# AndrewCullacino/handwritten-chinese-ocr-samples

Hardware: AMD Instinct MI355X
Metric: text-lines/sec (1x128x2000 synth) greedy decode (higher is better)
Workload: dtype f16 (f32 accumulate); 1 GPU; BASELINE configs[1]: 64 x 1x128x2000 uint8 lines, random-init hctr checkpoint (C=7358), forward + greedy CTC decode, labels to host; global_lines=64, lines_per_gpu=64, width=2000, classes=7358, checkpoint=random, parallelism=batch-shard x1

## Files before the change

### handwritten-chinese-ocr-samples_amd/csrc/engine.cpp

```cpp
#include "../../include/hctr_hip.h"
#include "kernels.h"

#include <algorithm>
#include <cfloat>
#include <cmath>
#include <cstdarg>
#include <cstdio>
#include <cstring>
#include <map>
#include <new>
#include <string>
#include <vector>

using namespace hctr;

namespace {

constexpr int kImgH = 128;
constexpr int kFeat = 2048;
constexpr double kBnEps = 1e-5;
constexpr int kStagePlanes[4] = {128, 256, 512, 512};
constexpr int kStageBlocks[4] = {2, 4, 5, 1};
constexpr int kStageH[5] = {128, 64, 32, 16, 8};
constexpr int64_t kDefaultMaxCols = 131072;

std::string g_create_error;

struct HostTensor {
    std::vector<float> data;
    std::vector<int64_t> shape;
    mutable bool used = false;
};

struct ConvW {
    half_t* w = nullptr;
    float* bias = nullptr;
    int cin = 0, cout = 0, coutPad = 0, taps = 0;
};

struct SeW {
    float* w1 = nullptr;
    float* w2 = nullptr;
    int c = 0;
};

struct BlockW {
    ConvW conv1, conv2, ds;
    SeW se;
    bool has_ds = false;
};

struct Workspace {
    int B = 0, W = 0, Wa = 0;
    void* img = nullptr;
    int32_t* widths = nullptr;
    half_t* s0 = nullptr;
    half_t* x[5] = {};
    half_t* p[5][3] = {};
    half_t* headin = nullptr;
    float* logits = nullptr;
    float* se_part = nullptr;
    float* se_scale = nullptr;
    float* se_border = nullptr;
    float* se_mean = nullptr;
    int32_t* se_counter = nullptr;
    int32_t* colidx = nullptr;
    float* amax_val = nullptr;
    int32_t* amax_idx = nullptr;
    int32_t* labels = nullptr;
    int32_t* lengths = nullptr;
    float* psum = nullptr;
    float* blank_logit = nullptr;
    float* row_thr = nullptr;
    int32_t* emit_cnt = nullptr;
    int32_t* emit_list = nullptr;
    double* esum = nullptr;
    int32_t* overflow = nullptr;
    int32_t* bm_idx = nullptr;
    float* bm_lp = nullptr;
    float* bm_bl = nullptr;
    float* bm_st = nullptr;
    int32_t* bm_cnt = nullptr;
    int32_t* tile_ctrs = nullptr;
    float* amax_val2 = nullptr;
    float* amax_abs = nullptr;
    float* col_margin = nullptr;
    float* col_abs = nullptr;
    float* line_guard = nullptr;
    int features = 0;
    bool split = false;
    bool aliased = false;
};

enum WsFeature { WS_S0 = 1, WS_LOGITS = 2, WS_BEAM = 4, WS_GUARD = 8 };

struct WeightSet {
    float* stem_w = nullptr;
    float* stem_b = nullptr;
// ... 311 lines not shown
    half_t* pool4[4] = {};
    auto layout = [&](bool alias) {
        ws = Workspace();
        ws.B = B; ws.W = W; ws.features = feat; ws.split = c->split; ws.Wa = Wa; ws.aliased = alias;
        off = 0;
        slots.clear();
        auto A = [&](auto** out, size_t count) {
            slots.emplace_back((void**)out, off);
            off += (std::max<size_t>(count * sizeof(**out), 16) + 255) & ~(size_t)255;
        };
        A((char**)&ws.img, cols * kImgH * 4);
        A(&ws.widths, (size_t)B);
        int cin = 64;
        size_t se_max = 0, pool_elems = 0;
        for (int s = 1; s <= 4; ++s) {
            const int H = kStageH[s], planes = kStagePlanes[s - 1];
            if (!alias) {
                A(&ws.x[s], (size_t)act_elems(B, H, Wa, cin * m));
                const int nbuf = (s == 4) ? 2 : 3;
                for (int i = 0; i < nbuf; ++i) A(&ws.p[s][i], (size_t)act_elems(B, H, Wa, planes * m));
            }
            pool_elems = std::max(pool_elems, (size_t)act_elems(B, H, Wa, std::max(cin, planes) * m));
            se_max = std::max(se_max, (size_t)B * (H / 8) * tilesW * planes);
            cin = planes;
        }
        if (alias)
            for (int i = 0; i < 4; ++i) A(&pool4[i], pool_elems);
        A(&ws.headin, cols * kFeat * m);
        A(&ws.se_part, se_max);
        A(&ws.se_scale, (size_t)B * 512);
        A(&ws.se_border, (size_t)B * 5 * 8 * 512);
        A(&ws.se_mean, (size_t)B * 512);
        A(&ws.se_counter, (size_t)B);
        A(&ws.colidx, cols);
        const size_t P = (size_t)head_parts_max(c);
        A(&ws.amax_val, cols * P);
        A(&ws.amax_idx, cols * P);
        A(&ws.labels, cols);
        A(&ws.lengths, (size_t)B);
        A(&ws.tile_ctrs, (size_t)64 * 8);
        if (feat & WS_S0) A(&ws.s0, (size_t)act_elems(B, 128, Wa, 64 * m));
        if (feat & WS_LOGITS) A(&ws.logits, cols * c->cpad);
        if (feat & WS_GUARD) {
            A(&ws.amax_val2, cols * P);
            A(&ws.amax_abs, cols * P);
            A(&ws.col_margin, cols);
            A(&ws.col_abs, cols);
            A(&ws.line_guard, (size_t)2 * B);
        }
        if (feat & WS_BEAM) {
            A(&ws.psum, P * cols);
            A(&ws.blank_logit, cols);
            A(&ws.row_thr, 2 * cols);
            A(&ws.emit_cnt, cols);
            A(&ws.esum, P * cols);
            A(&ws.overflow, (size_t)1);
            A(&ws.bm_idx, cols * kBeamMaxK);
            A(&ws.bm_lp, cols * kBeamMaxK);
            A(&ws.bm_bl, cols);
            A(&ws.bm_st, 2 * cols);
            A(&ws.bm_cnt, cols);
            A(&ws.emit_list, cols * kBeamCap * 2);
        }
    };
    bool alias = c->ws_alias == 1;
    layout(alias);
// ... 15 lines not shown
        c->arena = nullptr; c->arena_cap = 0;
        c->ws = Workspace();
        const size_t want = off + off / 16;
        void* p = nullptr;
        hipError_t e = hipMalloc(&p, want);
        if (e != hipSuccess) e = hipMalloc(&p, off);
        if (e != hipSuccess)
            return fail(c, HCTR_ERR_NOMEM, "hipMalloc(%zu bytes) for the workspace of %d lines x %d columns failed: %s", off,
                        B, W, hipGetErrorString(e));
        c->arena = (char*)p;
        c->arena_cap = e == hipSuccess && want >= off ? want : off;
        ++c->arena_reallocs;
        fresh = true;
    }
    for (auto& sl : slots) *sl.first = c->arena + sl.second;
    if (ws.aliased) {
        for (int s = 1; s <= 4; ++s) {
            ws.x[s] = pool4[0];
            for (int i = 0; i < ((s == 4) ? 2 : 3); ++i) ws.p[s][i] = pool4[1 + i];
        }
    }
    if (c->ws.aliased != ws.aliased) same_shape = false;
    auto zero_act = [&](half_t* p, int H, int C) { return launch_zero_borders(p, B, H, W, Wa, C * m, c->stream); };
    if (fresh || !same_shape) {
        int ci = 64;
        for (int s = 1; s <= 4 && !ws.aliased; ++s) {
            const int H = kStageH[s], planes = kStagePlanes[s - 1];
            HIP_TRY(c, zero_act(ws.x[s], H, ci));
            const int nbuf = (s == 4) ? 2 : 3;
            for (int i = 0; i < nbuf; ++i) HIP_TRY(c, zero_act(ws.p[s][i], H, planes));
            ci = planes;
        }
        HIP_TRY(c, hipMemsetAsync(ws.se_counter, 0, (size_t)B * 4, c->stream));
        ++c->ws_recarves;
    }
    if (ws.s0 && (fresh || !same_shape || !c->ws.s0)) HIP_TRY(c, zero_act(ws.s0, 128, 64));
    c->ws = ws;
    return HCTR_OK;
}

struct Prof {
    hctr_ctx* c;
    bool on;
    explicit Prof(hctr_ctx* ctx) : c(ctx), on(ctx->profiling) {}
    hipEvent_t ev() {
        if (c->ev_used == c->ev_pool.size()) {
            hipEvent_t e;
            (void)hipEventCreate(&e);
            c->ev_pool.push_back(e);
        }
        return c->ev_pool[c->ev_used++];
    }
    void begin(const char* name) {
        if (!on) return;
        ProfEntry pe{name, ev(), ev()};
        (void)hipEventRecord(pe.e0, c->stream);
        c->prof.push_back(pe);
    }
    void end() {
        if (!on) return;
        (void)hipEventRecord(c->prof.back().e1, c->stream);
    }
};

inline void prof_reset(hctr_ctx* c) {
    if (c->profiling) { c->prof.clear(); c->ev_used = 0; }
// ... 50 lines not shown
    if (ds) {
        if (tile != TILE_HALO4 || !se_scale || resid || ds->cin % kBK != 0 || ds->coutPad != cw.coutPad)
            return fail(c, HCTR_ERR_STATE, "conv %s: downsample fusion not applicable", name);
        a.ds_x = ds_in; a.ds_w = ds->w; a.ds_bias = ds->bias; a.ds_cin = ds->cin;
        a.ds_in_sh = ws.Wa * ds->cin;
        a.ds_in_sb = (int64_t)(in.H + 2) * ws.Wa * ds->cin;
    }
    a.mtiles = ws.B * a.tilesH * a.tilesW;
    a.ntiles = cw.coutPad / conv_tile_couts(tile);
    if (c->persist_dynamic && c->conv_seq < 64) a.tile_counter = ws.tile_ctrs + 8 * c->conv_seq++;
    if (c->stamp_buf && c->stamp_layer == name && (tile == TILE_HALO4 || tile == TILE_HALO4_8x32) &&
        (int64_t)a.mtiles * a.ntiles <= c->stamp_cap) {
        a.stamps = c->stamp_buf;
        c->stamp_n = (int64_t)a.mtiles * a.ntiles;
    }
    static const char* dbg_layer = getenv("HCTR_DBG_LAYER");
    if (dbg_layer && strcmp(dbg_layer, name) == 0)
        if (const char* e = getenv("HCTR_DBG")) a.dbg = atoi(e);
    pf.begin(name);
    if (stem_img_f32 >= 0) {
        if (tile != TILE_64x256 || cw.taps != 9 || cw.cin != 64 || cw.coutPad != 64 || c->split)
            return fail(c, HCTR_ERR_STATE, "conv %s: stem fusion not applicable", name);
        a.img = ws.img; a.img_f32 = stem_img_f32; a.img_widths = stem_widths ? ws.widths : nullptr;
        a.stem_w = c->wts().stem_w; a.stem_b = c->wts().stem_b;
        HIP_TRY(c, launch_stem_conv0_2(a, c->stream));
    } else {
        HIP_TRY(c, launch_conv(a, tile, cw.taps, false, c->stream));
    }
    pf.end();
    return HCTR_OK;
}

int run_block(hctr_ctx* c, Prof& pf, const std::string& name, const BlockW& bw, ActDesc in, half_t* t,
              half_t* o, half_t* r, int planes) {
    const Workspace& ws = c->ws;
    const int H = in.H;
    auto tiles_of = [&](const ConvW& cw) {
        const ConvTile t = pick_tile(c, cw, H);
        return (H / conv_tile_rows(t)) * ((ws.W + conv_tile_cols(t) - 1) / conv_tile_cols(t));
    };
    const float inv_hw = 1.0f / ((float)H * (float)ws.W);
    const half_t* res = in.p;
    const bool fuse_ds = bw.has_ds && c->fuse_ds && (c->fuse_se || c->split) && bw.ds.cin % kBK == 0 &&
                         pick_tile(c, bw.conv2, H) == TILE_HALO4;
    if (bw.has_ds && !fuse_ds) {
        c->out_class = 4;
        TRY(run_conv(c, pf, (name + ".downsample").c_str(), bw.ds, in, r, H, false, false, nullptr, false));
        res = r;
    }
    if (c->fuse_se || c->split) {
        const int tiles1 = tiles_of(bw.conv1);
        c->out_class = 2;
        TRY(run_conv(c, pf, (name + ".conv1").c_str(), bw.conv1, in, t, H, true, false, ws.se_part, false));
        c->out_class = 4;
        pf.begin((name + ".se_stats").c_str());
        HIP_TRY(c, launch_se_border(t, ws.B, H, ws.W, ws.Wa, planes, c->split, ws.se_part, tiles1, ws.se_border, c->stream));
        pf.end();
        pf.begin((name + ".se_scale").c_str());
        HIP_TRY(c, launch_se_premean(ws.se_border, t, bw.conv2.w, bw.conv2.bias, ws.B, H, ws.W, ws.Wa, planes,
                                     bw.conv2.coutPad, c->split, ws.se_mean, bw.se.w1, bw.se.w2, ws.se_scale,
                                     ws.se_counter, c->stream));
        pf.end();
        if (fuse_ds)
            TRY(run_conv(c, pf, (name + ".conv2+se+ds").c_str(), bw.conv2, ActDesc{t, H, planes}, o, H, true, false,
                         nullptr, false, ws.se_scale, nullptr, &bw.ds, in.p));
        else
            TRY(run_conv(c, pf, (name + ".conv2+se").c_str(), bw.conv2, ActDesc{t, H, planes}, o, H, true, false,
                         nullptr, false, ws.se_scale, res));
        return HCTR_OK;
    }
    c->out_class = 2;
    TRY(run_conv(c, pf, (name + ".conv1").c_str(), bw.conv1, in, t, H, true, false, nullptr, false));
    c->out_class = 4;
    TRY(run_conv(c, pf, (name + ".conv2").c_str(), bw.conv2, ActDesc{t, H, planes}, o, H, false, false,
                 ws.se_part, false));
    const int tiles = tiles_of(bw.conv2);
    pf.begin((name + ".se_fc").c_str());
    HIP_TRY(c, launch_se_fc(ws.se_part, tiles, bw.se.w1, bw.se.w2, ws.se_scale, ws.B, planes, inv_hw, c->stream));
    pf.end();
    pf.begin((name + ".se_apply").c_str());
    HIP_TRY(c, launch_se_apply(o, res, ws.se_scale, (int64_t)(H + 2) * ws.Wa * planes, ws.B, planes, c->stream));
    pf.end();
    return HCTR_OK;
}

enum HeadMode { HEAD_LOGITS = 0, HEAD_ARGMAX = 1, HEAD_BEAM = 2 };

int ws_need(const hctr_ctx* c, HeadMode mode, bool guarded = false) {
    int need = 0;
    if (mode == HEAD_LOGITS) need |= WS_LOGITS;
    if (mode == HEAD_BEAM) need |= WS_BEAM;
    if (!(c->fuse_stem && !c->split)) need |= WS_S0;
    if (guarded) need |= WS_GUARD;
    return need;
}

void head_args(hctr_ctx* c, ConvArgs* out, ConvTile* tile) {
    const Workspace& ws = c->ws;
    ConvArgs a{};
    a.x = ws.headin; a.w = c->wts().head.w; a.bias = c->wts().head.bias; a.y = ws.logits;
    a.Cin = c->wts().head.cin; a.Cout = c->num_classes; a.CoutPad = c->cpad;
    a.M = (int64_t)ws.B * ws.W; a.ldo = c->cpad;
    *tile = (c->big_tiles && c->cpad % 256 == 0) ? TILE_256x256 : TILE_128x128;
    const int hbm = *tile == TILE_256x256 ? 256 : 128;
    a.mtiles = (int)((a.M + hbm - 1) / hbm); a.ntiles = c->cpad / hbm;
    *out = a;
}

int run_forward(hctr_ctx* c, int img_f32, bool have_widths, HeadMode mode = HEAD_LOGITS, bool guarded = false) {
    if ((c->ws.features & ws_need(c, mode, guarded)) != ws_need(c, mode, guarded) || c->ws.split != c->split)
        return fail(c, HCTR_ERR_STATE, "workspace lacks a part this forward needs (ensure_workspace before staging)");
    Workspace& ws = c->ws;
    const WeightSet& wt = c->wts();
    if (!wt.built) return fail(c, HCTR_ERR_STATE, "the weight set of this precision mode is not resident");
    Prof pf(c);
    if (c->persist_dynamic) {
        HIP_TRY(c, hipMemsetAsync(ws.tile_ctrs, 0, 64 * 8 * 4, c->stream));
        c->conv_seq = 0;
    }
    auto zero_stage = [&](int s, bool input, bool blocks) -> int {
        if (!ws.aliased) return HCTR_OK;
        const int H = kStageH[s], planes = kStagePlanes[s - 1], cin_s = s == 1 ? 64 : kStagePlanes[s - 2];
        const int mm = c->chm();
        pf.begin("zero_borders");
        if (input) HIP_TRY(c, launch_zero_borders(ws.x[s], ws.B, H, ws.W, ws.Wa, cin_s * mm, c->stream));
        for (int i = 0; blocks && i < ((s == 4) ? 2 : 3); ++i)
            HIP_TRY(c, launch_zero_borders(ws.p[s][i], ws.B, H, ws.W, ws.Wa, planes * mm, c->stream));
        pf.end();
        return HCTR_OK;
    };
    TRY(zero_stage(1, true, true));
    c->out_class = 8;
    if (c->fuse_stem && !c->split) {
        TRY(run_conv(c, pf, "stem+conv0_2+pool", wt.conv0_2, ActDesc{nullptr, 128, 64}, ws.x[1], 64, true, true, nullptr,
                     false, nullptr, nullptr, nullptr, nullptr, img_f32 ? 1 : 0, have_widths));
    } else {
        pf.begin("stem.conv0_1");
        HIP_TRY(c, launch_stem(ws.img, img_f32, have_widths ? ws.widths : nullptr, wt.stem_w, wt.stem_b, ws.s0, ws.B,
                               ws.W, ws.Wa, c->split ? ((c->x3_mask & 8) ? 1 : 2) : 0, c->stream));
        pf.end();
        TRY(run_conv(c, pf, "conv0_2+pool", wt.conv0_2, ActDesc{ws.s0, 128, 64}, ws.x[1], 64, true, true, nullptr, false));
    }
    int cin = 64;
    for (int s = 1; s <= 4; ++s) {
        const int H = kStageH[s], planes = kStagePlanes[s - 1];
        ActDesc cur{ws.x[s], H, cin};
        int ci = -1;
        for (size_t i = 0; i < wt.blocks[s - 1].size(); ++i) {
            const BlockW& bw = wt.blocks[s - 1][i];
            char nm[48];
            snprintf(nm, sizeof(nm), "block%d.%zu", s, i);
            const int ti = ci < 0 ? 0 : (ci + 1) % 3, oi = ci < 0 ? 1 : (ci + 2) % 3;
            if (bw.has_ds && ci >= 0) return fail(c, HCTR_ERR_STATE, "downsample only expected on a stage's first block");
            TRY(run_block(c, pf, nm, bw, cur, ws.p[s][ti], ws.p[s][oi], bw.has_ds ? ws.p[s][2] : nullptr, planes));
            cur = ActDesc{ws.p[s][oi], H, planes};
            ci = oi;
        }
        char nm[32];
        snprintf(nm, sizeof(nm), "conv%d+pool", s);
        c->out_class = s < 4 ? 8 : 16;
        if (s < 4) {
            TRY(zero_stage(s + 1, true, false));
            TRY(run_conv(c, pf, nm, wt.stage_conv[s - 1], cur, ws.x[s + 1], H / 2, true, true, nullptr, false));
            TRY(zero_stage(s + 1, false, true));
        } else
            TRY(run_conv(c, pf, nm, wt.stage_conv[s - 1], cur, ws.headin, H / 2, true, true, nullptr, true));
        cin = planes;
    }
    ConvArgs a;
    ConvTile htile;
    head_args(c, &a, &htile);
    auto line_guard = [&]() -> int {
        pf.begin("line_guard");
        HIP_TRY(c, launch_line_guard(ws.col_margin, ws.col_abs, ws.B, ws.W, ws.line_guard, c->stream));
        pf.end();
        return HCTR_OK;
    };
    if (mode == HEAD_ARGMAX || mode == HEAD_BEAM) {
        a.y = nullptr;
        a.amax_val = ws.amax_val;
        a.amax_idx = ws.amax_idx;
        if (guarded) { a.amax_val2 = ws.amax_val2; a.amax_abs = ws.amax_abs; }
        if (mode == HEAD_BEAM) { a.psum = ws.psum; a.blank_logit = ws.blank_logit; }
        pf.begin(mode == HEAD_BEAM ? "head.linear+partials" : "head.linear+argmax");
        HIP_TRY(c, launch_conv(a, htile, 1, true, c->stream));
        pf.end();
        if (mode == HEAD_BEAM && !guarded) return HCTR_OK;
// ... 1129 lines not shown
            return 0;
        }
        if (!out || !c->stamp_buf) return fail(c, HCTR_ERR_STATE, "stamping not armed");
        const int64_t n = std::min(c->stamp_n, cap_wgs);
        if (hipMemcpy(out, c->stamp_buf, (size_t)n * 128, hipMemcpyDeviceToHost) != hipSuccess)
            return fail(c, HCTR_ERR_HIP, "stamp copy");
        return n;
    });
}

int64_t hctr_debug_activation(hctr_ctx* c, const char* name, float* out, int64_t cap, int* Cout, int* Hout) {
    return guard<int64_t>(c, [&]() -> int64_t {
        if (!c || !name) return HCTR_ERR_ARG;
        const Workspace& ws = c->ws;
        if (ws.B == 0) return fail(c, HCTR_ERR_STATE, "no forward has run");
        const half_t* p = nullptr;
        int H = 0, C = 0;
        bool head = false;
        const std::string n(name);
        if (n == "conv0_1") {
            if (!ws.s0) return fail(c, HCTR_ERR_STATE, "conv0_1 is fused into conv0_2 (no buffer): use HCTR_FUSE_STEM=0");
            p = ws.s0; H = 128; C = 64;
        }
        else if (n == "stage0") { p = ws.x[1]; H = 64; C = 64; }
        else if (n == "stage1") { p = ws.x[2]; H = 32; C = 128; }
        else if (n == "stage2") { p = ws.x[3]; H = 16; C = 256; }
        else if (n == "stage3") { p = ws.x[4]; H = 8; C = 512; }
        else if (n == "stage4") { p = ws.headin; H = 4; C = 512; head = true; }
        else if (n.size() == 4 && n[0] == 'p' && n[2] == '.' && n[1] >= '1' && n[1] <= '4' && n[3] >= '0' && n[3] <= '2') {
            const int st = n[1] - '0', bi = n[3] - '0';
            p = ws.p[st][bi]; H = kStageH[st]; C = kStagePlanes[st - 1];
            if (!p) return fail(c, HCTR_ERR_ARG, "buffer %s not allocated", name);
        }
        else return fail(c, HCTR_ERR_ARG, "unknown activation '%s'", name);
        if (ws.aliased && !(n == "stage3" || n == "stage4" || (n.size() == 4 && n[0] == 'p' && n[1] == '4')))
            return fail(c, HCTR_ERR_STATE, "activation '%s' was overwritten by a later stage: the stages share their buffers "
                        "in this workspace layout (HCTR_WS_ALIAS=0 keeps every stage's own)", name);
        const int64_t total = (int64_t)ws.B * C * H * ws.W;
        if (Cout) *Cout = C;
        if (Hout) *Hout = H;
        if (!out || cap < total) return total;
        HIP_TRY(c, hipStreamSynchronize(c->stream));
        const int m = ws.split ? 3 : 1;
        const int64_t elems = head ? (int64_t)ws.B * ws.W * kFeat * m : act_elems(ws.B, H, ws.Wa, C * m);
        std::vector<half_t> host((size_t)elems);
        HIP_TRY(c, hipMemcpy(host.data(), p, (size_t)elems * sizeof(half_t), hipMemcpyDeviceToHost));
        for (int b = 0; b < ws.B; ++b)
            for (int ch = 0; ch < C; ++ch)
                for (int h = 0; h < H; ++h)
                    for (int w = 0; w < ws.W; ++w) {
                        const int64_t src = head ? (((int64_t)b * ws.W + w) * 4 + h) * (512 * m) + ch
                                                 : (((int64_t)b * (H + 2) + h + 1) * ws.Wa + w + 1) * (C * m) + ch;
                        float v = (float)host[(size_t)src];
                        if (m == 3) v += (float)host[(size_t)src + C];
                        out[(((int64_t)b * C + ch) * H + h) * ws.W + w] = v;
                    }
        return total;
    });
}

}
```

### handwritten-chinese-ocr-samples_amd/csrc/kernels.h

```cpp
#pragma once
#include <hip/hip_runtime.h>
#include <stdint.h>

namespace hctr {

typedef _Float16 half_t;

constexpr int kTileW = 16;
constexpr int kBK = 64;

struct ConvArgs {
    const half_t* x;
    const half_t* w;
    const float* bias;
    void* y;
    float* se_part;
    const float* se_scale;
    const half_t* resid;
    int H, W;
    int Cin, Cout, CoutPad;
    int tilesW, tilesH;
    int64_t in_sb;
    int in_sh;
    int64_t out_sb;
// ... 24 lines not shown
    const float* stem_b;
    int split;
    int drop_lo;
    const half_t* ds_x;
    const half_t* ds_w;
    const float* ds_bias;
    int ds_cin;
    int ds_in_sh;
    int64_t ds_in_sb;
    int32_t* tile_counter;
    unsigned long long* stamps;
    int dbg;
};

enum ConvTile { TILE_64x256 = 0, TILE_128x128 = 1, TILE_256x256 = 2, TILE_HALO4 = 3, TILE_HALO4_8x32 = 4 };
inline int conv_tile_rows(ConvTile t) { return (t == TILE_128x128 || t == TILE_HALO4_8x32) ? 8 : 16; }
inline int conv_tile_cols(ConvTile t) { return t == TILE_HALO4_8x32 ? 32 : 16; }
inline int conv_tile_couts(ConvTile t) {
    return t == TILE_64x256 ? 64 : (t == TILE_256x256 ? 256 : 128);
}

hipError_t launch_conv(const ConvArgs& a, ConvTile tile, int taps, bool linear_f32, hipStream_t s);
constexpr int kLinearWN = 2;
hipError_t launch_argmax_partials(const float* val, const int32_t* cls, int P, int64_t M, int32_t* idx, hipStream_t s,
                                  const float* val2 = nullptr, const float* absp = nullptr, float* margin = nullptr,
                                  float* rowabs = nullptr);
hipError_t launch_row_guard(const float* logits, int64_t ld, int64_t M, int C, float* margin, float* rowabs, hipStream_t s);
hipError_t launch_line_guard(const float* margin, const float* rowabs, int B, int W, float* out, hipStream_t s);
size_t conv_lds_bytes(ConvTile tile);

hipError_t launch_stem_conv0_2(const ConvArgs& a, hipStream_t s);

hipError_t launch_zero_borders(half_t* p, int B, int H, int W, int Wa, int C, hipStream_t s);

hipError_t launch_stem(const void* img, int img_f32, const int32_t* widths_dev, const float* w9,
                       const float* bias, half_t* y, int B, int W, int Wa, int split, hipStream_t s);

hipError_t launch_se_border(const half_t* t, int B, int H, int W, int Wa, int C, int split, const float* tsum_part,
                            int tiles, float* out, hipStream_t s);
hipError_t launch_se_premean(const float* border, const half_t* t, const half_t* w, const float* bias, int B, int H,
                             int W, int Wa, int C, int CoutPad, int split, float* mean, const float* w1,
                             const float* w2, float* scale, int32_t* counter, hipStream_t s);

hipError_t launch_se_fc(const float* se_part, int tiles_per_img, const float* w1, const float* w2,
                        float* scale, int B, int C, float inv_hw, hipStream_t s);

hipError_t launch_se_apply(half_t* o, const half_t* r, const float* scale, int64_t img_elems,
                           int B, int C, hipStream_t s);

hipError_t launch_argmax_rows(const float* logits, int64_t ld, int64_t M, int C, int32_t* idx,
                              int tB, int tW, hipStream_t s);

constexpr int kBeamCap = 256;
constexpr int kBeamMaxK = 32;
hipError_t launch_beam_thresholds(const float* pmax, const float* psum, int P, int64_t M, int k, double cand_thresh,
                                  int want_candidates, float* row_thr, int32_t* emit_cnt, hipStream_t s);
hipError_t launch_beam_select(const float* row_thr, const int32_t* emit_cnt, const int32_t* emit_list, int cap,
                              const double* esum, int P, const float* blank_logit, int B, int W, int k,
                              double cand_thresh, int32_t* topk_idx, float* topk_logp, float* blank_logp,
                              float* stats, int32_t* cand_count, int32_t* overflow, hipStream_t s);
hipError_t launch_beam_candidates(const int32_t* emit_cnt, const int32_t* emit_list, int cap, const float* stats,
                                  int B, int W, double cand_thresh, const int64_t* cand_off, int32_t* cand_idx,
                                  float* cand_logp, hipStream_t s);

hipError_t launch_ctc_collapse(const int32_t* idx, int B, int W, int C, int32_t* labels,
                               int32_t* lengths, hipStream_t s);

hipError_t launch_logits_to_wbc(const float* logits, int64_t ld, int B, int W, int C, float* out,
                                int Bfull, int b0, hipStream_t s);
hipError_t launch_wbc_to_rows(const float* wbc, int B, int W, int C, float* rows, int64_t ld,
                              hipStream_t s);

hipError_t launch_row_topk(const float* logits, int64_t ld, int B, int W, int C, int k, double thresh,
                           int32_t* topk_idx, float* topk_logp, float* blank_logp, float* stats,
                           int32_t* cand_count, hipStream_t s);
// ... 43 lines not shown
```

### handwritten-chinese-ocr-samples_amd/csrc/kernels.hip

```cpp
#include "kernels.h"

#include <cstdlib>

namespace hctr {

typedef _Float16 f16x8 __attribute__((ext_vector_type(8)));
typedef float f32x4 __attribute__((ext_vector_type(4)));
typedef float f32x2 __attribute__((ext_vector_type(2)));
typedef _Float16 f16x2 __attribute__((ext_vector_type(2)));
typedef uint32_t u32x4 __attribute__((ext_vector_type(4)));
typedef void __attribute__((address_space(3))) * lptr_t;

__device__ __forceinline__ void glds16_asm(const char* gsrc, char* lds_dst) {
    const uint32_t lds = (uint32_t)(uintptr_t)((lptr_t)lds_dst);
    uint32_t keep;
    asm volatile("s_mov_b32 %0, m0\n\ts_mov_b32 m0, %2\n\ts_nop 0\n\tglobal_load_lds_dwordx4 %1, off\n\ts_mov_b32 m0, %0"
                 : "=&s"(keep)
                 : "v"(gsrc), "s"(lds)
                 : "memory");
}

template <int CTRL>
__device__ __forceinline__ float dpp_f32(float v) {
    return __builtin_bit_cast(float, __builtin_amdgcn_update_dpp(0, __builtin_bit_cast(int, v), CTRL, 0xF, 0xF, true));
// ... 1568 lines not shown
    float win[3][3];
#pragma unroll
    for (int r = 0; r < 2; ++r)
#pragma unroll
        for (int d = 0; d < 3; ++d) win[r + 1][d] = pixel(h0 - 1 + r, w - 1 + d);
    const int cs = split ? 192 : 64;
    for (int r = 0; r < kStemRows; ++r) {
        const int h = h0 + r;
#pragma unroll
        for (int d = 0; d < 3; ++d) {
            win[0][d] = win[1][d];
            win[1][d] = win[2][d];
            win[2][d] = pixel(h + 1, w - 1 + d);
        }
        f16x8 o, ol;
#pragma unroll
        for (int e = 0; e < 8; ++e) {
            float sv = bs[e];
#pragma unroll
            for (int t = 0; t < 9; ++t) sv = fmaf(wt[e][t], win[t / 3][t % 3], sv);
            sv = fmaxf(sv, 0.f);
            o[e] = (half_t)sv;
            ol[e] = split == 2 ? (half_t)0.f : (half_t)(sv - (float)o[e]);
        }
        half_t* dst = y + (((int64_t)b * 130 + h + 1) * Wa + (w + 1)) * cs + cg * 8;
        *(f16x8*)dst = o;
        if (split) {
            *(f16x8*)(dst + 64) = ol;
            *(f16x8*)(dst + 128) = o;
        }
    }
}

__global__ __launch_bounds__(256) void zero_borders_kernel(half_t* __restrict__ p, int H, int W, int Wa, int C) {
    const int row = blockIdx.x, b = blockIdx.y;
    u32x4* r = (u32x4*)(p + ((int64_t)b * (H + 2) + row) * (int64_t)Wa * C);
    const int vpp = C >> 3;
    const u32x4 z = {0u, 0u, 0u, 0u};
    if (row == 0 || row == H + 1) {
        for (int i = threadIdx.x; i < Wa * vpp; i += 256) r[i] = z;
        return;
    }
    for (int i = threadIdx.x; i < vpp; i += 256) r[i] = z;
    const int first = (W + 1) * vpp, n = (Wa - W - 1) * vpp;
    for (int i = threadIdx.x; i < n; i += 256) r[first + i] = z;
}

hipError_t launch_zero_borders(half_t* p, int B, int H, int W, int Wa, int C, hipStream_t s) {
    if (B == 0) return hipSuccess;
    if (C % 8 != 0 || Wa < W + 2) return hipErrorInvalidValue;
    hipLaunchKernelGGL(zero_borders_kernel, dim3(H + 2, B), dim3(256), 0, s, p, H, W, Wa, C);
    return hipGetLastError();
}

hipError_t launch_stem(const void* img, int img_f32, const int32_t* widths_dev, const float* w9,
                       const float* bias, half_t* y, int B, int W, int Wa, int split, hipStream_t s) {
    if (B == 0) return hipSuccess;
    hipLaunchKernelGGL(stem_kernel, dim3((W + 31) / 32, 128 / kStemRows, B), dim3(256), 0, s, img, img_f32, widths_dev,
                       w9, bias, y, B, W, Wa, split);
    return hipGetLastError();
}

constexpr int kS2Halo = 32768;
constexpr int kS2Patch = 32768 + kHaloBytes;
constexpr int kS2Lds = kS2Patch + 20 * 20 * 4;

__global__ __launch_bounds__(256, 2) void stem_conv0_2_kernel(const ConvArgs a) {
    constexpr int JT = 4, S = kHaloCols;
    extern __shared__ __attribute__((aligned(16))) char smem[];
    const int tid = threadIdx.x;
    const int lane = tid & 63;
    const int wv = __builtin_amdgcn_readfirstlane(tid >> 6);
    const int total = a.mtiles;
    int lin;
    {
        const int id = blockIdx.x, xcd = id & 7, sl = id >> 3;
        const int qd = total >> 3, r = total & 7;
        lin = (xcd < r ? xcd * (qd + 1) : r * (qd + 1) + (xcd - r) * qd) + sl;
    }
    const int tw = lin % a.tilesW;
    const int t2 = lin / a.tilesW;
    const int th = t2 % a.tilesH;
    const int img = t2 / a.tilesH;
    const int W = a.W;

// ... 96 lines not shown
            const char* be = hb + v0;
            const char* bo = hb + (v0 ^ 64);
            const char* wtile = smem + (st & 1) * 16384 + tt * 8192;
#pragma unroll
            for (int ks = 0; ks < 2; ++ks) {
                f16x8 af[JT], bf[4];
#pragma unroll
                for (int n = 0; n < 4; ++n) bf[n] = *(const f16x8*)((((n & 1) ^ ks) ? bo : be) + n * (S * 128));
#pragma unroll
                for (int j = 0; j < JT; ++j) af[j] = *(const f16x8*)(wtile + j * 2048 + (ks ? aoff1 : aoff0));
                __builtin_amdgcn_s_setprio(1);
#pragma unroll
                for (int j = 0; j < JT; ++j)
#pragma unroll
                    for (int n = 0; n < 4; ++n)
                        acc[j][n] = __builtin_amdgcn_mfma_f32_16x16x32_f16(af[j], bf[n], acc[j][n], 0, 0, 0);
                __builtin_amdgcn_s_setprio(0);
            }
        }
    }
    conv_epilogue<1, 4, JT, false, false>(a, acc, smem, tid, lane, 0, wv, 0, lin, img, th, tw, th * 16 + wrow, tw * 16);
}

hipError_t launch_stem_conv0_2(const ConvArgs& a, hipStream_t s) {
    if (a.mtiles == 0) return hipSuccess;
    static bool done[64] = {};
    hipError_t e0 = raise_lds_limit((const void*)stem_conv0_2_kernel, kS2Lds, done);
    if (e0 != hipSuccess) return e0;
    hipLaunchKernelGGL(stem_conv0_2_kernel, dim3(a.mtiles), dim3(256), kS2Lds, s, a);
    return hipGetLastError();
}

constexpr int kBorderSeg = 8;

__global__ __launch_bounds__(256) void se_border_kernel(const half_t* __restrict__ t, int H, int W, int Wa, int C,
                                                        int split, const float* __restrict__ tsum_part, int tiles,
                                                        float* __restrict__ out) {
    __shared__ float red[256 * 8];
    const int b = blockIdx.x, job = blockIdx.y;
    const int seg = blockIdx.z;
    if (job == 4) {
        const int per = (tiles + kBorderSeg - 1) / kBorderSeg;
        const int t0 = seg * per, t1 = t0 + per < tiles ? t0 + per : tiles;
        for (int ci = threadIdx.x; ci < C; ci += 256) {
            const float* p = tsum_part + (int64_t)b * tiles * C + ci;
            float s0 = 0.f, s1 = 0.f;
            int i = t0;
            for (; i + 1 < t1; i += 2) { s0 += p[(int64_t)i * C]; s1 += p[(int64_t)(i + 1) * C]; }
            if (i < t1) s0 += p[(int64_t)i * C];
            out[(((int64_t)b * 5 + 4) * kBorderSeg + seg) * C + ci] = s0 + s1;
        }
        return;
    }
    const int cv = C >> 3;
    const int v = threadIdx.x % cv, lanes = 256 / cv, p0 = threadIdx.x / cv;
    const int cs = split ? 3 * C : C;
    const half_t* img = t + (int64_t)b * (H + 2) * Wa * cs;
    const int count = job < 2 ? W : H;
    const int per = (count + kBorderSeg - 1) / kBorderSeg;
    const int pbeg = seg * per, pend = pbeg + per < count ? pbeg + per : count;
    float acc[8] = {0, 0, 0, 0, 0, 0, 0, 0};
    if (threadIdx.x < lanes * cv) {
        auto addr = [&](int p) {
            const int h = job == 0 ? 0 : (job == 1 ? H - 1 : p);
            const int w = job == 2 ? 0 : (job == 3 ? W - 1 : p);
            return img + ((int64_t)(h + 1) * Wa + (w + 1)) * cs + v * 8;
        };
        int p = pbeg + p0;
        for (; p + 3 * lanes < pend; p += 4 * lanes) {
            f16x8 x[4], xl[4];
#pragma unroll
            for (int u = 0; u < 4; ++u) {
                const half_t* px = addr(p + u * lanes);
// ... 6 lines not shown
                for (int e = 0; e < 8; ++e) acc[e] += (float)x[u][e];
                if (split) {
#pragma unroll
                    for (int e = 0; e < 8; ++e) acc[e] += (float)xl[u][e];
                }
            }
        }
        for (; p < pend; p += lanes) {
            const half_t* px = addr(p);
            const f16x8 x = *(const f16x8*)px;
#pragma unroll
            for (int e = 0; e < 8; ++e) acc[e] += (float)x[e];
            if (split) {
                const f16x8 xl = *(const f16x8*)(px + C);
#pragma unroll
                for (int e = 0; e < 8; ++e) acc[e] += (float)xl[e];
            }
        }
    }
#pragma unroll
    for (int e = 0; e < 8; ++e) red[threadIdx.x * 8 + e] = acc[e];
    __syncthreads();
    if (threadIdx.x < cv) {
        float s[8] = {0, 0, 0, 0, 0, 0, 0, 0};
        for (int l = 0; l < lanes; ++l)
#pragma unroll
            for (int e = 0; e < 8; ++e) s[e] += red[(l * cv + threadIdx.x) * 8 + e];
#pragma unroll
        for (int e = 0; e < 8; ++e)
            out[(((int64_t)b * 5 + job) * kBorderSeg + seg) * C + threadIdx.x * 8 + e] = s[e];
    }
}

hipError_t launch_se_border(const half_t* t, int B, int H, int W, int Wa, int C, int split, const float* tsum_part,
                            int tiles, float* out, hipStream_t s) {
    hipLaunchKernelGGL(se_border_kernel, dim3(B, 5, kBorderSeg), dim3(256), 0, s, t, H, W, Wa, C, split, tsum_part, tiles, out);
    return hipGetLastError();
}

__global__ __launch_bounds__(256) void se_premean_kernel(const float* __restrict__ border,
                                                         const half_t* __restrict__ t,
                                                         const half_t* __restrict__ w,
                                                         const float* __restrict__ bias, int H, int W, int Wa,
                                                         int C, int CoutPad, int split,
                                                         float* __restrict__ mean, const float* __restrict__ w1,
                                                         const float* __restrict__ w2, float* __restrict__ scale,
                                                         int32_t* __restrict__ counter) {
    __shared__ float S[9 * 512];
    __shared__ float part[256];
    __shared__ int last_flag;
    const int b = blockIdx.x, cg = blockIdx.y;
    const int cs = split ? 3 * C : C;
    const half_t* img = t + (int64_t)b * (H + 2) * Wa * cs;
    for (int ci = threadIdx.x; ci < C; ci += 256) {
        float bsum[5];
#pragma unroll
        for (int jb = 0; jb < 5; ++jb) {
            const float* bd = border + (((int64_t)b * 5 + jb) * kBorderSeg) * C + ci;
            float sv = 0.f;
#pragma unroll
            for (int sg = 0; sg < kBorderSeg; ++sg) sv += bd[(int64_t)sg * C];
            bsum[jb] = sv;
        }
        const float R0 = bsum[0], RL = bsum[1], C0 = bsum[2], CL = bsum[3], T = bsum[4];
        auto px = [&](int hp, int wp) {
            const half_t* q = img + ((int64_t)hp * Wa + wp) * cs + ci;
            return split ? (float)q[0] + (float)q[C] : (float)q[0];
        };
        const float t00 = px(1, 1), t0L = px(1, W), tL0 = px(H, 1), tLL = px(H, W);
#pragma unroll
        for (int tap = 0; tap < 9; ++tap) {
            const int dy = tap / 3 - 1, dx = tap % 3 - 1;
            float sv = T;
            if (dy == 1) sv -= R0;
            if (dy == -1) sv -= RL;
            if (dx == 1) sv -= C0;
            if (dx == -1) sv -= CL;
            if (dy == 1 && dx == 1) sv += t00;
            if (dy == 1 && dx == -1) sv += t0L;
            if (dy == -1 && dx == 1) sv += tL0;
            if (dy == -1 && dx == -1) sv += tLL;
            S[tap * C + ci] = sv;
        }
    }
    __syncthreads();
    const int cl = threadIdx.x & 63, slice = threadIdx.x >> 6;
    const int jj = (cl >> 5) * 2 + ((cl >> 2) & 1), qq = (cl >> 3) & 3, ii = cl & 3;
    const int srow = jj * 16 + qq * 4 + ii;
    float acc = 0.f;
    const int kper = 9 * C / 4;
    int kk0 = slice * kper;
    const int kend = (slice + 1) * kper;
    for (; kk0 + 64 <= kend; kk0 += 64) {
        f16x8 wv8[8], wl8[8];
// ... 6 lines not shown
            if (split) wl8[u] = *(const f16x8*)(wr + 2 * C);
        }
#pragma unroll
        for (int u = 0; u < 8; ++u) {
            const int kk = kk0 + u * 8;
            const int tap = kk / C, ci = kk - tap * C;
            if (split) {
#pragma unroll
                for (int e = 0; e < 8; ++e) acc = fmaf((float)wv8[u][e] + (float)wl8[u][e], S[tap * C + ci + e], acc);
            } else {
#pragma unroll
                for (int e = 0; e < 8; ++e) acc = fmaf((float)wv8[u][e], S[tap * C + ci + e], acc);
            }
        }
    }
    for (int kk = kk0; kk < kend; kk += 8) {
        const int tap = kk / C, ci = kk - tap * C;
        const half_t* wr = w + ((int64_t)tap * CoutPad + cg * 64 + srow) * cs + ci;
        const f16x8 wv = *(const f16x8*)wr;
        if (split) {
            const f16x8 wl = *(const f16x8*)(wr + 2 * C);
#pragma unroll
            for (int e = 0; e < 8; ++e) acc = fmaf((float)wv[e] + (float)wl[e], S[tap * C + ci + e], acc);
        } else {
#pragma unroll
            for (int e = 0; e < 8; ++e) acc = fmaf((float)wv[e], S[tap * C + ci + e], acc);
        }
    }
    part[threadIdx.x] = acc;
    __syncthreads();
    if (threadIdx.x < 64) {
        const float tot = (part[threadIdx.x] + part[64 + threadIdx.x]) + (part[128 + threadIdx.x] + part[192 + threadIdx.x]);
        const int c = cg * 64 + threadIdx.x;
        mean[(int64_t)b * C + c] = bias[c] + tot / ((float)H * (float)W);
    }
    asm volatile("s_waitcnt vmcnt(0)" ::: "memory");
    __syncthreads();
    if (threadIdx.x == 0) {
        __builtin_amdgcn_fence(__ATOMIC_RELEASE, "agent");
        asm volatile("s_waitcnt vmcnt(0)" ::: "memory");
        const int ticket = __hip_atomic_fetch_add(counter + b, 1, __ATOMIC_RELAXED, __HIP_MEMORY_SCOPE_AGENT);
        const int last = ticket == (int)gridDim.y - 1;
        if (last) {
            __hip_atomic_store(counter + b, 0, __ATOMIC_RELAXED, __HIP_MEMORY_SCOPE_AGENT);
            __builtin_amdgcn_fence(__ATOMIC_ACQUIRE, "agent");
            asm volatile("s_waitcnt vmcnt(0)" ::: "memory");
        }
        last_flag = last;
    }
    __syncthreads();
    if (!last_flag) return;
    float* mean_s = S;
    float* hid = S + 512;
    for (int c = threadIdx.x; c < C; c += 256)
        mean_s[c] = __hip_atomic_load(mean + (int64_t)b * C + c, __ATOMIC_RELAXED, __HIP_MEMORY_SCOPE_AGENT);
    __syncthreads();
    const int R = C / 16;
    {
        const int r = threadIdx.x >> 3, l = threadIdx.x & 7;
        float sv = 0.f;
        if (r < R)
            for (int c = l; c < C; c += 8) sv = fmaf(w1[r * C + c], mean_s[c], sv);
        sv += __shfl_xor(sv, 1);
        sv += __shfl_xor(sv, 2);
        sv += __shfl_xor(sv, 4);
        if (r < R && l == 0) hid[r] = fmaxf(sv, 0.f);
    }
    __syncthreads();
    for (int c = threadIdx.x; c < C; c += 256) {
        float sv = 0.f;
        for (int r = 0; r < R; ++r) sv = fmaf(w2[c * R + r], hid[r], sv);
        scale[(int64_t)b * C + c] = 1.f / (1.f + expf(-sv));
    }
}

hipError_t launch_se_premean(const float* border, const half_t* t, const half_t* w, const float* bias, int B, int H,
                             int W, int Wa, int C, int CoutPad, int split, float* mean, const float* w1,
                             const float* w2, float* scale, int32_t* counter, hipStream_t s) {
    if (C > 512 || C % 64 != 0) return hipErrorInvalidValue;
    hipLaunchKernelGGL(se_premean_kernel, dim3(B, C / 64), dim3(256), 0, s, border, t, w, bias, H, W, Wa, C, CoutPad,
                       split, mean, w1, w2, scale, counter);
    return hipGetLastError();
}

__global__ __launch_bounds__(256) void se_fc_kernel(const float* __restrict__ part, int tiles,
                                                    const float* __restrict__ w1,
                                                    const float* __restrict__ w2,
                                                    float* __restrict__ scale, int C, float inv_hw) {
    __shared__ float mean[512];
    __shared__ float hid[32];
    const int b = blockIdx.x;
    const int R = C / 16;
    for (int c = threadIdx.x; c < C; c += 256) {
        const float* p = part + (int64_t)b * tiles * C + c;
        float s0 = 0.f, s1 = 0.f, s2 = 0.f, s3 = 0.f;
        int t = 0;
        for (; t + 3 < tiles; t += 4) {
            s0 += p[(int64_t)t * C];
            s1 += p[(int64_t)(t + 1) * C];
            s2 += p[(int64_t)(t + 2) * C];
            s3 += p[(int64_t)(t + 3) * C];
        }
        for (; t < tiles; ++t) s0 += p[(int64_t)t * C];
        mean[c] = ((s0 + s1) + (s2 + s3)) * inv_hw;
    }
    __syncthreads();
    {
        const int r = threadIdx.x >> 3, l = threadIdx.x & 7;
        float s = 0.f;
        if (r < R)
            for (int c = l; c < C; c += 8) s = fmaf(w1[r * C + c], mean[c], s);
        s += __shfl_xor(s, 1);
        s += __shfl_xor(s, 2);
        s += __shfl_xor(s, 4);
// ... 983 lines not shown
```

Baseline: 512.9 lines/s.

## Fuse SE border and premean kernels into one ticketed persistent-style kernel

```diff
diff --git a/handwritten-chinese-ocr-samples_amd/csrc/engine.cpp b/handwritten-chinese-ocr-samples_amd/csrc/engine.cpp
--- a/handwritten-chinese-ocr-samples_amd/csrc/engine.cpp
+++ b/handwritten-chinese-ocr-samples_amd/csrc/engine.cpp
@@ -21,6 +21,8 @@
 constexpr double kBnEps = 1e-5;
 constexpr int kStagePlanes[4] = {128, 256, 512, 512};
 constexpr int kStageBlocks[4] = {2, 4, 5, 1};
+constexpr int kSeTapPerStage = 5;
+constexpr int kSeTapSlots = 4 * kSeTapPerStage;
 constexpr int kStageH[5] = {128, 64, 32, 16, 8};
 constexpr int64_t kDefaultMaxCols = 131072;
 
@@ -64,6 +66,8 @@
     float* se_border = nullptr;
     float* se_mean = nullptr;
     int32_t* se_counter = nullptr;
+    float* se_scale_tap = nullptr;
+    int32_t* se_tick_a = nullptr;
     int32_t* colidx = nullptr;
     float* amax_val = nullptr;
     int32_t* amax_idx = nullptr;
@@ -441,6 +445,8 @@
         A(&ws.se_border, (size_t)B * 5 * 8 * 512);
         A(&ws.se_mean, (size_t)B * 512);
         A(&ws.se_counter, (size_t)B);
+        A(&ws.se_tick_a, (size_t)B + 1);
+        A(&ws.se_scale_tap, (size_t)kSeTapSlots * B * 512);
         A(&ws.colidx, cols);
         const size_t P = (size_t)head_parts_max(c);
         A(&ws.amax_val, cols * P);
@@ -522,6 +528,7 @@
             ci = planes;
         }
         HIP_TRY(c, hipMemsetAsync(ws.se_counter, 0, (size_t)B * 4, c->stream));
+        HIP_TRY(c, hipMemsetAsync(ws.se_tick_a, 0, ((size_t)B + 1) * 4, c->stream));
         ++c->ws_recarves;
     }
     if (ws.s0 && (fresh || !same_shape || !c->ws.s0)) HIP_TRY(c, zero_act(ws.s0, 128, 64));
@@ -638,7 +645,7 @@
 }
 
 int run_block(hctr_ctx* c, Prof& pf, const std::string& name, const BlockW& bw, ActDesc in, half_t* t,
-              half_t* o, half_t* r, int planes) {
+              half_t* o, half_t* r, int planes, int tap_slot) {
     const Workspace& ws = c->ws;
     const int H = in.H;
     auto tiles_of = [&](const ConvW& cw) {
@@ -659,13 +666,11 @@
         c->out_class = 2;
         TRY(run_conv(c, pf, (name + ".conv1").c_str(), bw.conv1, in, t, H, true, false, ws.se_part, false));
         c->out_class = 4;
-        pf.begin((name + ".se_stats").c_str());
-        HIP_TRY(c, launch_se_border(t, ws.B, H, ws.W, ws.Wa, planes, c->split, ws.se_part, tiles1, ws.se_border, c->stream));
-        pf.end();
         pf.begin((name + ".se_scale").c_str());
-        HIP_TRY(c, launch_se_premean(ws.se_border, t, bw.conv2.w, bw.conv2.bias, ws.B, H, ws.W, ws.Wa, planes,
-                                     bw.conv2.coutPad, c->split, ws.se_mean, bw.se.w1, bw.se.w2, ws.se_scale,
-                                     ws.se_counter, c->stream));
+        HIP_TRY(c, launch_se_scale(t, ws.se_part, tiles1, ws.se_border, bw.conv2.w, bw.conv2.bias, ws.B, H, ws.W, ws.Wa,
+                                   planes, bw.conv2.coutPad, c->split, ws.se_mean, bw.se.w1, bw.se.w2, ws.se_scale,
+                                   ws.se_scale_tap + (size_t)tap_slot * ws.B * 512, ws.se_tick_a, ws.se_counter,
+                                   c->stream));
         pf.end();
         if (fuse_ds)
             TRY(run_conv(c, pf, (name + ".conv2+se+ds").c_str(), bw.conv2, ActDesc{t, H, planes}, o, H, true, false,
@@ -728,10 +733,12 @@
         if (!ws.aliased) return HCTR_OK;
         const int H = kStageH[s], planes = kStagePlanes[s - 1], cin_s = s == 1 ? 64 : kStagePlanes[s - 2];
         const int mm = c->chm();
+        ZeroBordersArgs za{};
+        int n = 0;
+        if (input) { za.p[n] = ws.x[s]; za.C[n++] = cin_s * mm; }
+        for (int i = 0; blocks && i < ((s == 4) ? 2 : 3); ++i) { za.p[n] = ws.p[s][i]; za.C[n++] = planes * mm; }
         pf.begin("zero_borders");
-        if (input) HIP_TRY(c, launch_zero_borders(ws.x[s], ws.B, H, ws.W, ws.Wa, cin_s * mm, c->stream));
-        for (int i = 0; blocks && i < ((s == 4) ? 2 : 3); ++i)
-            HIP_TRY(c, launch_zero_borders(ws.p[s][i], ws.B, H, ws.W, ws.Wa, planes * mm, c->stream));
+        HIP_TRY(c, launch_zero_borders_multi(za, n, ws.B, H, ws.W, ws.Wa, c->stream));
         pf.end();
         return HCTR_OK;
     };
@@ -758,7 +765,9 @@
             snprintf(nm, sizeof(nm), "block%d.%zu", s, i);
             const int ti = ci < 0 ? 0 : (ci + 1) % 3, oi = ci < 0 ? 1 : (ci + 2) % 3;
             if (bw.has_ds && ci >= 0) return fail(c, HCTR_ERR_STATE, "downsample only expected on a stage's first block");
-            TRY(run_block(c, pf, nm, bw, cur, ws.p[s][ti], ws.p[s][oi], bw.has_ds ? ws.p[s][2] : nullptr, planes));
+            if (i >= (size_t)kSeTapPerStage) return fail(c, HCTR_ERR_STATE, "more blocks in a stage than scale tap slots");
+            TRY(run_block(c, pf, nm, bw, cur, ws.p[s][ti], ws.p[s][oi], bw.has_ds ? ws.p[s][2] : nullptr, planes,
+                          (s - 1) * kSeTapPerStage + (int)i));
             cur = ActDesc{ws.p[s][oi], H, planes};
             ci = oi;
         }
@@ -1954,6 +1963,21 @@
             p = ws.p[st][bi]; H = kStageH[st]; C = kStagePlanes[st - 1];
             if (!p) return fail(c, HCTR_ERR_ARG, "buffer %s not allocated", name);
         }
+        else if (n.size() == 14 && n.compare(0, 5, "block") == 0 && n[6] == '.' && n.compare(8, 6, ".scale") == 0 &&
+                 n[5] >= '1' && n[5] <= '4' && n[7] >= '0' && n[7] < '0' + kSeTapPerStage) {
+            const int st = n[5] - '0', bi = n[7] - '0';
+            if (!(c->fuse_se || ws.split) || bi >= (int)c->wts().blocks[st - 1].size())
+                return fail(c, HCTR_ERR_ARG, "no scale tap '%s' in this configuration", name);
+            const int Cs = kStagePlanes[st - 1];
+            const int64_t total = (int64_t)ws.B * Cs;
+            if (Cout) *Cout = Cs;
+            if (Hout) *Hout = 1;
+            if (!out || cap < total) return total;
+            HIP_TRY(c, hipStreamSynchronize(c->stream));
+            const float* src = ws.se_scale_tap + (size_t)((st - 1) * kSeTapPerStage + bi) * ws.B * 512;
+            HIP_TRY(c, hipMemcpy2D(out, (size_t)Cs * 4, src, 512 * 4, (size_t)Cs * 4, (size_t)ws.B, hipMemcpyDeviceToHost));
+            return total;
+        }
         else return fail(c, HCTR_ERR_ARG, "unknown activation '%s'", name);
         if (ws.aliased && !(n == "stage3" || n == "stage4" || (n.size() == 4 && n[0] == 'p' && n[1] == '4')))
             return fail(c, HCTR_ERR_STATE, "activation '%s' was overwritten by a later stage: the stages share their buffers "
diff --git a/handwritten-chinese-ocr-samples_amd/csrc/kernels.h b/handwritten-chinese-ocr-samples_amd/csrc/kernels.h
--- a/handwritten-chinese-ocr-samples_amd/csrc/kernels.h
+++ b/handwritten-chinese-ocr-samples_amd/csrc/kernels.h
@@ -80,15 +80,19 @@
 hipError_t launch_stem_conv0_2(const ConvArgs& a, hipStream_t s);
 
 hipError_t launch_zero_borders(half_t* p, int B, int H, int W, int Wa, int C, hipStream_t s);
+struct ZeroBordersArgs {
+    half_t* p[4];
+    int C[4];
+};
+hipError_t launch_zero_borders_multi(const ZeroBordersArgs& a, int n, int B, int H, int W, int Wa, hipStream_t s);
 
 hipError_t launch_stem(const void* img, int img_f32, const int32_t* widths_dev, const float* w9,
                        const float* bias, half_t* y, int B, int W, int Wa, int split, hipStream_t s);
 
-hipError_t launch_se_border(const half_t* t, int B, int H, int W, int Wa, int C, int split, const float* tsum_part,
-                            int tiles, float* out, hipStream_t s);
-hipError_t launch_se_premean(const float* border, const half_t* t, const half_t* w, const float* bias, int B, int H,
-                             int W, int Wa, int C, int CoutPad, int split, float* mean, const float* w1,
-                             const float* w2, float* scale, int32_t* counter, hipStream_t s);
+hipError_t launch_se_scale(const half_t* t, const float* tsum_part, int tiles, float* border, const half_t* w,
+                           const float* bias, int B, int H, int W, int Wa, int C, int CoutPad, int split, float* mean,
+                           const float* w1, const float* w2, float* scale, float* scale_tap, int32_t* tick_a,
+                           int32_t* counter, hipStream_t s);
 
 hipError_t launch_se_fc(const float* se_part, int tiles_per_img, const float* w1, const float* w2,
                         float* scale, int B, int C, float inv_hw, hipStream_t s);
diff --git a/handwritten-chinese-ocr-samples_amd/csrc/kernels.hip b/handwritten-chinese-ocr-samples_amd/csrc/kernels.hip
--- a/handwritten-chinese-ocr-samples_amd/csrc/kernels.hip
+++ b/handwritten-chinese-ocr-samples_amd/csrc/kernels.hip
@@ -1624,8 +1624,11 @@
     }
 }
 
-__global__ __launch_bounds__(256) void zero_borders_kernel(half_t* __restrict__ p, int H, int W, int Wa, int C) {
+__global__ __launch_bounds__(256) void zero_borders_kernel(ZeroBordersArgs a, int H, int W, int Wa) {
     const int row = blockIdx.x, b = blockIdx.y;
+    half_t* p = a.p[blockIdx.z];
+    if (!p) return;
+    const int C = a.C[blockIdx.z];
     u32x4* r = (u32x4*)(p + ((int64_t)b * (H + 2) + row) * (int64_t)Wa * C);
     const int vpp = C >> 3;
     const u32x4 z = {0u, 0u, 0u, 0u};
@@ -1638,11 +1641,19 @@
     for (int i = threadIdx.x; i < n; i += 256) r[first + i] = z;
 }
 
+hipError_t launch_zero_borders_multi(const ZeroBordersArgs& a, int n, int B, int H, int W, int Wa, hipStream_t s) {
+    if (B == 0 || n == 0) return hipSuccess;
+    if (n < 0 || n > 4 || Wa < W + 2) return hipErrorInvalidValue;
+    for (int i = 0; i < n; ++i)
+        if (a.p[i] && a.C[i] % 8 != 0) return hipErrorInvalidValue;
+    hipLaunchKernelGGL(zero_borders_kernel, dim3(H + 2, B, n), dim3(256), 0, s, a, H, W, Wa);
+    return hipGetLastError();
+}
+
 hipError_t launch_zero_borders(half_t* p, int B, int H, int W, int Wa, int C, hipStream_t s) {
-    if (B == 0) return hipSuccess;
-    if (C % 8 != 0 || Wa < W + 2) return hipErrorInvalidValue;
-    hipLaunchKernelGGL(zero_borders_kernel, dim3(H + 2, B), dim3(256), 0, s, p, H, W, Wa, C);
-    return hipGetLastError();
+    ZeroBordersArgs a{};
+    a.p[0] = p; a.C[0] = C;
+    return launch_zero_borders_multi(a, 1, B, H, W, Wa, s);
 }
 
 hipError_t launch_stem(const void* img, int img_f32, const int32_t* widths_dev, const float* w9,
@@ -1805,13 +1816,13 @@
 }
 
 constexpr int kBorderSeg = 8;
-
-__global__ __launch_bounds__(256) void se_border_kernel(const half_t* __restrict__ t, int H, int W, int Wa, int C,
-                                                        int split, const float* __restrict__ tsum_part, int tiles,
-                                                        float* __restrict__ out) {
-    __shared__ float red[256 * 8];
-    const int b = blockIdx.x, job = blockIdx.y;
-    const int seg = blockIdx.z;
+constexpr int kSeUnits = 5 * kBorderSeg;
+constexpr int kSeLag = 2;
+constexpr long long kSeSpinTicks = 1ll << 27;
+
+__device__ __forceinline__ void se_phase_a(const half_t* __restrict__ t, int H, int W, int Wa, int C, int split,
+                                           const float* __restrict__ tsum_part, int tiles, float* out, float* red,
+                                           int b, int job, int seg) {
     if (job == 4) {
         const int per = (tiles + kBorderSeg - 1) / kBorderSeg;
         const int t0 = seg * per, t1 = t0 + per < tiles ? t0 + per : tiles;
@@ -1884,24 +1895,10 @@
     }
 }
 
-hipError_t launch_se_border(const half_t* t, int B, int H, int W, int Wa, int C, int split, const float* tsum_part,
-                            int tiles, float* out, hipStream_t s) {
-    hipLaunchKernelGGL(se_border_kernel, dim3(B, 5, kBorderSeg), dim3(256), 0, s, t, H, W, Wa, C, split, tsum_part, tiles, out);
-    return hipGetLastError();
-}
-
-__global__ __launch_bounds__(256) void se_premean_kernel(const float* __restrict__ border,
-                                                         const half_t* __restrict__ t,
-                                                         const half_t* __restrict__ w,
-                                                         const float* __restrict__ bias, int H, int W, int Wa,
-                                                         int C, int CoutPad, int split,
-                                                         float* __restrict__ mean, const float* __restrict__ w1,
-                                                         const float* __restrict__ w2, float* __restrict__ scale,
-                                                         int32_t* __restrict__ counter) {
-    __shared__ float S[9 * 512];
-    __shared__ float part[256];
-    __shared__ int last_flag;
-    const int b = blockIdx.x, cg = blockIdx.y;
+__device__ __forceinline__ void se_phase_b(const float* border, const half_t* __restrict__ t,
+                                           const half_t* __restrict__ w, const float* __restrict__ bias, int H, int W,
+                                           int Wa, int C, int CoutPad, int split, float* mean, float* S, float* part,
+                                           int b, int cg, bool poison) {
     const int cs = split ? 3 * C : C;
     const half_t* img = t + (int64_t)b * (H + 2) * Wa * cs;
     for (int ci = threadIdx.x; ci < C; ci += 256) {
@@ -1911,7 +1908,8 @@
             const float* bd = border + (((int64_t)b * 5 + jb) * kBorderSeg) * C + ci;
             float sv = 0.f;
 #pragma unroll
-            for (int sg = 0; sg < kBorderSeg; ++sg) sv += bd[(int64_t)sg * C];
+            for (int sg = 0; sg < kBorderSeg; ++sg)
+                sv += __hip_atomic_load(bd + (int64_t)sg * C, __ATOMIC_RELAXED, __HIP_MEMORY_SCOPE_AGENT);
             bsum[jb] = sv;
         }
         const float R0 = bsum[0], RL = bsum[1], C0 = bsum[2], CL = bsum[3], T = bsum[4];
@@ -1984,24 +1982,88 @@
     if (threadIdx.x < 64) {
         const float tot = (part[threadIdx.x] + part[64 + threadIdx.x]) + (part[128 + threadIdx.x] + part[192 + threadIdx.x]);
         const int c = cg * 64 + threadIdx.x;
-        mean[(int64_t)b * C + c] = bias[c] + tot / ((float)H * (float)W);
-    }
+        const float m = bias[c] + tot / ((float)H * (float)W);
+        mean[(int64_t)b * C + c] = poison ? __builtin_nanf("") : m;
+    }
+}
+
+__global__ __launch_bounds__(256) void se_scale_kernel(const half_t* __restrict__ t,
+                                                       const float* __restrict__ tsum_part, int tiles, float* border,
+                                                       const half_t* __restrict__ w, const float* __restrict__ bias,
+                                                       int B, int H, int W, int Wa, int C, int CoutPad, int split,
+                                                       float* mean, const float* __restrict__ w1,
+                                                       const float* __restrict__ w2, float* __restrict__ scale,
+                                                       float* __restrict__ scale_tap, int32_t* tick_a,
+                                                       int32_t* counter) {
+    __shared__ float S[9 * 512];
+    __shared__ float part[256];
+    __shared__ int item_s, flag_s;
+    const int G = C / 64;
+    if (threadIdx.x == 0) {
+        const int it = __hip_atomic_fetch_add(tick_a + B, 1, __ATOMIC_RELAXED, __HIP_MEMORY_SCOPE_AGENT);
+        if (it == (int)gridDim.x - 1) __hip_atomic_store(tick_a + B, 0, __ATOMIC_RELAXED, __HIP_MEMORY_SCOPE_AGENT);
+        item_s = it;
+    }
+    __syncthreads();
+    const int L = B < kSeLag ? B : kSeLag;
+    int k = item_s, b, unit;
+    if (k < L * kSeUnits) {
+        b = k / kSeUnits; unit = k - b * kSeUnits;
+    } else {
+        k -= L * kSeUnits;
+        const int mid = (B - L) * (G + kSeUnits);
+        if (k < mid) {
+            const int i = k / (G + kSeUnits), r = k - i * (G + kSeUnits);
+            if (r < G) { b = i; unit = -r - 1; }
+            else { b = i + L; unit = r - G; }
+        } else {
+            k -= mid;
+            b = B - L + k / G; unit = -(k % G) - 1;
+        }
+    }
+    if (unit >= 0) {
+        se_phase_a(t, H, W, Wa, C, split, tsum_part, tiles, border, S, b, unit / kBorderSeg, unit % kBorderSeg);
+        asm volatile("s_waitcnt vmcnt(0)" ::: "memory");
+        __syncthreads();
+        if (threadIdx.x == 0) {
+            __builtin_amdgcn_fence(__ATOMIC_RELEASE, "agent");
+            asm volatile("s_waitcnt vmcnt(0)" ::: "memory");
+            (void)__hip_atomic_fetch_add(tick_a + b, 1, __ATOMIC_RELAXED, __HIP_MEMORY_SCOPE_AGENT);
+        }
+        return;
+    }
+    const int cg = -unit - 1;
+    if (threadIdx.x == 0) {
+        const long long t0 = wall_clock64();
+        int ok = 1;
+        while (__hip_atomic_load(tick_a + b, __ATOMIC_RELAXED, __HIP_MEMORY_SCOPE_AGENT) < kSeUnits) {
+            __builtin_amdgcn_s_sleep(8);
+            if (wall_clock64() - t0 > kSeSpinTicks) { ok = 0; break; }
+        }
+        __builtin_amdgcn_fence(__ATOMIC_ACQUIRE, "agent");
+        asm volatile("s_waitcnt vmcnt(0)" ::: "memory");
+        flag_s = ok;
+    }
+    __syncthreads();
+    const bool poison = !flag_s;
+    se_phase_b(border, t, w, bias, H, W, Wa, C, CoutPad, split, mean, S, part, b, cg, poison);
     asm volatile("s_waitcnt vmcnt(0)" ::: "memory");
     __syncthreads();
     if (threadIdx.x == 0) {
         __builtin_amdgcn_fence(__ATOMIC_RELEASE, "agent");
         asm volatile("s_waitcnt vmcnt(0)" ::: "memory");
         const int ticket = __hip_atomic_fetch_add(counter + b, 1, __ATOMIC_RELAXED, __HIP_MEMORY_SCOPE_AGENT);
-        const int last = ticket == (int)gridDim.y - 1;
+        const int last = ticket == G - 1;
         if (last) {
             __hip_atomic_store(counter + b, 0, __ATOMIC_RELAXED, __HIP_MEMORY_SCOPE_AGENT);
+            __hip_atomic_store(tick_a + b, 0, __ATOMIC_RELAXED, __HIP_MEMORY_SCOPE_AGENT);
             __builtin_amdgcn_fence(__ATOMIC_ACQUIRE, "agent");
             asm volatile("s_waitcnt vmcnt(0)" ::: "memory");
         }
-        last_flag = last;
+        flag_s = last;
     }
     __syncthreads();
-    if (!last_flag) return;
+    if (!flag_s) return;
     float* mean_s = S;
     float* hid = S + 512;
     for (int c = threadIdx.x; c < C; c += 256)
@@ -2022,16 +2084,20 @@
     for (int c = threadIdx.x; c < C; c += 256) {
         float sv = 0.f;
         for (int r = 0; r < R; ++r) sv = fmaf(w2[c * R + r], hid[r], sv);
-        scale[(int64_t)b * C + c] = 1.f / (1.f + expf(-sv));
-    }
-}
-
-hipError_t launch_se_premean(const float* border, const half_t* t, const half_t* w, const float* bias, int B, int H,
-                             int W, int Wa, int C, int CoutPad, int split, float* mean, const float* w1,
-                             const float* w2, float* scale, int32_t* counter, hipStream_t s) {
-    if (C > 512 || C % 64 != 0) return hipErrorInvalidValue;
-    hipLaunchKernelGGL(se_premean_kernel, dim3(B, C / 64), dim3(256), 0, s, border, t, w, bias, H, W, Wa, C, CoutPad,
-                       split, mean, w1, w2, scale, counter);
+        const float sc = 1.f / (1.f + expf(-sv));
+        scale[(int64_t)b * C + c] = sc;
+        scale_tap[(int64_t)b * 512 + c] = sc;
+    }
+}
+
+hipError_t launch_se_scale(const half_t* t, const float* tsum_part, int tiles, float* border, const half_t* w,
+                           const float* bias, int B, int H, int W, int Wa, int C, int CoutPad, int split, float* mean,
+                           const float* w1, const float* w2, float* scale, float* scale_tap, int32_t* tick_a,
+                           int32_t* counter, hipStream_t s) {
+    if (B == 0) return hipSuccess;
+    if (C > 512 || C % 64 != 0 || (int64_t)B * (kSeUnits + C / 64) > INT32_MAX) return hipErrorInvalidValue;
+    hipLaunchKernelGGL(se_scale_kernel, dim3(B * (kSeUnits + C / 64)), dim3(256), 0, s, t, tsum_part, tiles, border, w,
+                       bias, B, H, W, Wa, C, CoutPad, split, mean, w1, w2, scale, scale_tap, tick_a, counter);
     return hipGetLastError();
 }
 
```

After: 499.8 lines/s. 2.6% lower.
